# mobilecoinofficial/grapevine

Hardware: AMD Instinct MI355X
Metric: oblivious CRUD req/s (node) at 2^24 msgs, 64K batch; % HBM peak (higher is better)
Workload: dtype u8

## Files before the change

grapevine_amd/csrc/gvs_engine.hip:

```cpp
#include <hip/hip_runtime.h>
#include <rccl/rccl.h>

#include <cmath>
#include <cstdio>
#include <cstdlib>
#include <cstring>
#include <new>
#include <string>
#include <thread>
#include <algorithm>
#include <vector>

#include "../../include/gvstore.h"
#include "../../include/gvstore_test.h"
#include "gvs_kernels.h"
#include "gvs_route.h"
#include "gvs_mtx.h"
#include "gvs_kv.h"
#include "gvs_omap.h"
#include "gvs_wire.h"
#include "gvs_sr25519.h"
#include "gvs_ed25519.h"
#include "gvs_chacha.h"
#include "gvs_spass.h"
// ... 281 lines not shown
    return GVS_ERR_INVALID_ARG;
  if (c->flags & ~(GVS_FLAG_AUTH_STORAGE | GVS_FLAG_ED25519_AUTH)) return GVS_ERR_INVALID_ARG;
  if ((c->flags & GVS_FLAG_AUTH_STORAGE) && c->mailbox_partition_slots > kSrAuth) return GVS_ERR_INVALID_ARG;
  if (c->rows_per_partition && (!is_pow2(c->rows_per_partition) ||
                                c->rows_per_partition < (uint32_t)kTile ||
                                c->rows_per_partition > (uint32_t)kRowsMax))
    return GVS_ERR_INVALID_ARG;
  if (c->shard_count > kShardsMax) return GVS_ERR_INVALID_ARG;
  if (c->route_capacity > c->max_batch) return GVS_ERR_INVALID_ARG;
  for (int i = 0; i < 2; ++i)
    if (c->reserved[i] != 0) return GVS_ERR_INVALID_ARG;
  if (c->expiry_per_batch &&
      (!is_pow2(c->expiry_per_batch) || c->expiry_per_batch > c->max_batch / 2))
    return GVS_ERR_INVALID_ARG;
  return GVS_OK;
}

static uint32_t auto_capacity(uint32_t B, uint32_t S) {
  if (S <= 1) return B;
  const double mu = std::ceil((double)B / S);
  uint64_t c = (uint64_t)std::ceil(mu + 8.0 * std::sqrt(mu) + 64.0);
  c = (c + 63) / 64 * 64;
  return (uint32_t)(c < B ? c : B);
}

static uint32_t shard_batch(uint64_t m) {
  uint64_t p2 = 1024;
  while (p2 < m) p2 <<= 1;
  const uint64_t r = (m + 8191) / 8192 * 8192;
  const uint64_t be = std::max<uint64_t>(1024, std::min(p2, r));
  return be > (1u << (kSeqBits - 1)) ? 0u : (uint32_t)be;
}

static uint32_t txn_slots(uint32_t B, uint32_t W, uint32_t S) {
  const double mu = (double)B / W;
  uint64_t c = (uint64_t)std::ceil(mu + 8.0 * std::sqrt(mu) + 16.0);
  c = (c + 7) / 8 * 8;
  if (c > S) c = S;
  if (c > B) c = B;
  if (c > kSlotMax) c = kSlotMax;
  return (uint32_t)c;
}

static bool expiry_fits(const gvs_config* c, bool sharded) {
  if (!c->expiry_per_batch) return true;
  uint32_t Be = c->max_batch;
  if (sharded) {
    const uint32_t S = c->shard_count ? c->shard_count : 1;
    const uint32_t C = c->route_capacity ? c->route_capacity : auto_capacity(c->max_batch, S);
    Be = shard_batch((uint64_t)S * C + c->expiry_per_batch);
    if (!Be) return false;
  }
  const uint32_t need = txn_slots(c->expiry_per_batch, c->mailbox_partitions, ~0u);
  return need <= txn_slots(Be, c->mailbox_partitions, kGroupMax);
}


static uint8_t gf_mul(uint8_t a, uint8_t b) {
  uint8_t p = 0;
  for (int i = 0; i < 8; ++i) {
    if (b & 1) p ^= a;
    a = (uint8_t)((a << 1) ^ ((a & 0x80) ? 0x1b : 0));
    b >>= 1;
  }
  return p;
}
// ... 93 lines not shown
  for (uint32_t t = 0; t < 4; ++t) sc.l3p[t] = ld32(kb + 1200 + 4 * t);
  sc.nhk = nullptr;
  sc.epoch = 0;
  sc.on = 1;
}

static SealCtx seal_of(const gvs_handle* h, const Engine& e) {
  SealCtx c = h->sc;
  c.epoch = e.epoch;
  return c;
}

static int engine_init(gvs_handle* h, Engine& e, uint32_t shard, uint32_t B) {
  const gvs_config* cfg = &h->cfg;
  e.shard = shard;
  e.N = cfg->msg_capacity;
  e.Q = cfg->mailbox_partitions;
  e.Sr = cfg->mailbox_partition_slots;
  e.R = (uint64_t)e.Q * e.Sr;
  e.B = B;
  e.logQ = log2u(e.Q);
  uint64_t S = cfg->rows_per_partition ? cfg->rows_per_partition : e.N / 4096;
  if (S < (uint64_t)kTile) S = kTile;
  if (S > (uint64_t)kRowsMax) S = kRowsMax;
  if (S > e.N) S = e.N;
  if (!is_pow2(S)) return GVS_ERR_INVALID_ARG;
  e.S = (uint32_t)S;
  e.W = (uint32_t)(e.N / S);
  e.nblk = B / 1024;
  e.ring_size = e.N + B;
  if (e.W + 1 > (uint32_t)kBinsMax) return GVS_ERR_INVALID_ARG;
  e.c = txn_slots(B, e.W, e.S);
  e.cm = txn_slots(B, e.Q, kGroupMax);
  e.X = cfg->expiry_per_batch;
  if (e.X) {
    e.xep = e.X >= e.W ? e.X / e.W : 1u;
    e.xk = e.X >= e.W ? 1u : e.W / e.X;
    if (e.xep > kXepMax) return GVS_ERR_INVALID_ARG;
  }
  e.kc.pk0 = ld64(cfg->secret_key);
  e.kc.pk1 = ld64(cfg->secret_key + 8);
  e.kc.hk0 = ld64(cfg->secret_key + 16);
  e.kc.hk1 = ld64(cfg->secret_key + 24);
  e.kc.tag = shard_tag(shard);
  e.kc.nshards = h->S;

#define A(ptr, n)                                \
  do {                                           \
    if (int r_ = dalloc_t(h, &e.ptr, (n))) return r_; \
  } while (0)
  const uint64_t E = kExtra;
  A(table, e.N * 64);
  A(mbox, e.R * 64);
  A(side, e.R);
  A(ring, e.ring_size);
  A(scal, 1);
  A(img, (B + E) * 64);
  A(types, B);
  A(ops, B);
  A(kinds, B);
  A(s1keys, B);
  A(m1out, B + E);
  A(pflag, B);
  A(pslot, B);
  A(bsum, 2 * e.nblk);
  A(cslot, B);
// ... 164 lines not shown
  h->rt.resize(n_src);
  for (uint32_t k = 0; k < n_eng; ++k) {
    const uint32_t shard = mode == kRccl ? cfg->shard_index : k;
    if (int rc = engine_init(h, h->eng[k], shard, h->Be)) return fail(rc);
  }
  for (uint32_t k = 0; k < n_src; ++k)
    if (int rc = router_init(h, h->rt[k])) return fail(rc);
  const uint64_t stage = (uint64_t)h->Bsub * (mode == kLocal ? h->S : 1u);
  if (int rc = dalloc_t(h, &h->in_stage, stage * kAbiU4)) return fail(rc);
  if (int rc = dalloc_t(h, &h->out_stage, stage * kAbiU4)) return fail(rc);
  if (mode == kRccl) {
    ncclUniqueId id;
    std::memcpy(&id, comm_id, sizeof id);
    ncclResult_t r = ncclCommInitRank(&h->comm, (int)h->S, id, (int)cfg->shard_index);
    if (r != ncclSuccess) {
      h->err = std::string("ncclCommInitRank: ") + ncclGetErrorString(r);
      h->comm = nullptr;
      return fail(GVS_ERR_DEVICE);
    }
  }
  *out = h;
  return GVS_OK;
}


static uint32_t lower_count(uint32_t n, uint32_t blk, uint32_t half) {
  return (n / blk) * half + std::min(n % blk, half);
}

template <typename K, int E>
static void sort_tiles(hipStream_t s, K* d, uint32_t n) {
  constexpr uint32_t L = 1024u * E;
  hipLaunchKernelGGL((k_bitonic_tile<K, E>), dim3(n / L), dim3(1024), 0, s, d, 0u, 1);
  for (uint32_t k = 2 * L; (k >> 1) < n; k <<= 1) {
    uint32_t j = k >> 1;
    for (; j >= 8 * L; j >>= 4) {
      const uint32_t nq = lower_count(n, 2 * j, j >> 3);
      hipLaunchKernelGGL(k_bitonic_global4<K>, dim3((nq + 255) / 256), dim3(256), 0, s, d, n, k, j, nq);
    }
    for (; j >= 2 * L; j >>= 2) {
      const uint32_t nq = lower_count(n, 2 * j, j >> 1);
      hipLaunchKernelGGL(k_bitonic_global2<K>, dim3((nq + 255) / 256), dim3(256), 0, s, d, n, k, j, nq);
    }
    if (j >= L) {
      const uint32_t np = lower_count(n, 2 * j, j);
      hipLaunchKernelGGL(k_bitonic_global<K>, dim3((np + 255) / 256), dim3(256), 0, s, d, n, k, j, np);
    }
    hipLaunchKernelGGL((k_bitonic_tile<K, E>), dim3(n / L), dim3(1024), 0, s, d, k, 0);
  }
}

template <typename K, int EMAX>
static int sort_keys(gvs_handle* h, K* d, uint32_t n) {
  if (n < 1024 || n % 1024) return GVS_ERR_INTERNAL;
  uint32_t e = EMAX;
  while ((n / 1024) % e) e >>= 1;
  switch (e) {
    case 1: sort_tiles<K, 1>(h->stream, d, n); break;
    case 2: sort_tiles<K, 2>(h->stream, d, n); break;
    case 4: sort_tiles<K, (EMAX < 4 ? EMAX : 4)>(h->stream, d, n); break;
    default: sort_tiles<K, EMAX>(h->stream, d, n); break;
  }
  GVS_HIP(h, hipGetLastError());
  return GVS_OK;
}

static MArgs margs(const gvs_handle* h, const Engine& e) {
  MArgs a{};
  a.sc = seal_of(h, e);
  a.te = h->te;
  a.btag = e.btag;
  a.keys = e.s1keys;
  a.mbox = e.mbox;
  a.side = e.side;
  a.m1out = e.m1out;
  a.rop = e.rop;
  a.rres = e.rres;
  a.scal = e.scal;
  a.Q = e.Q;
  a.Sr = e.Sr;
// ... 81 lines not shown

static int phase_a2(gvs_handle* h, Engine& e, const uint4* d_in, uint32_t stride, uint32_t n) {
  hipStream_t s = h->stream;
  const uint32_t B = e.B, nblk = e.nblk;
  e.stamp_run = e.stamp_next++;
  if (e.stamp_next == kNone) e.stamp_next = 1;
  const uint32_t xbase = B - e.X;
  e.gtx = e.gtxb[e.gsel];
  e.gsel ^= 1u;
  const bool fuse = e.m2_pending;
  hipLaunchKernelGGL(k_copy, dim3(B / (4 * kCopyPerWave)), dim3(256), 0, s, d_in, stride, n, B, e.img, e.types,
                     (const uint4*)(e.X ? e.xb2[e.par ^ 1] : nullptr), xbase);
  mark(h, "copy");
  {
    MetaArgs a{e.img, e.types, e.ops, e.kinds, e.s1keys, n, B, e.Q, e.logQ, e.N, e.kc, xbase, e.idn};
    hipLaunchKernelGGL(k_meta, dim3(B / 256), dim3(256), 0, s, a);
  }
  mark(h, "meta");
  if (int r = sort_keys<Key128, 1>(h, e.s1keys, B)) return r;
  mark(h, "sort_s1");
  {
    GtxArgs a{e.s1keys, e.ops, e.mpos, e.gtx, e.gtx_agg, e.gtx_carry, fuse ? e.gscal : e.scal,
              B,        e.Q,   e.logQ, e.cm,  B / kScanT, e.stamp_run};
    a.mpid = e.mpid;
    hipLaunchKernelGGL(k_scan_a<GtxOp>, dim3(B / kScanT), dim3(kScanT), 0, s, a);
    hipLaunchKernelGGL(k_scan_b<GtxOp>, dim3(1), dim3(kScanT), 0, s, a);
    hipLaunchKernelGGL(k_scan_c<GtxOp>, dim3(B / kScanT), dim3(kScanT), 0, s, a);
  }
  mark(h, "gtx");
  if (h->auth) {
    hipLaunchKernelGGL(k_m1a, dim3(e.Q), dim3(256), (e.cm + 1) * sizeof(GroupM) + GVS_MA_EXTRA_LDS, s, margs2(h, e));
  } else if (fuse) {
    M21Args fa{e.m2_args, margs2(h, e), &e.gscal->error};
    hipLaunchKernelGGL(k_m21x, dim3(e.Q), dim3(256), e.Sr * sizeof(uint4) + 2 * (e.cm + 1) * sizeof(GroupM), s,
                       fa);
    hipLaunchKernelGGL(k_err_fold, dim3(1), dim3(64), 0, s, e.scal, &e.gscal->error);
    e.m2_pending = false;
  } else {
    hipLaunchKernelGGL(k_m1x<false>, dim3(e.Q), dim3(256), (e.cm + 1) * sizeof(GroupM), s, margs2(h, e));
  }
  {
    M1rArgs a{};
    vscan_fields(a, e);
    a.mpos = e.mpos;
    a.ops = e.ops;
    a.msnapp = e.msnapp;
    a.mpid = e.mpid;
    a.m1out = e.m1out;
    a.N = e.N;
    a.kc = e.kc;
    vscan_abc<M1rOp>(s, a);
    hipLaunchKernelGGL(k_m1r_c, dim3(a.nvb), dim3(256), 0, s, a);
  }
  mark(h, "m1");
  {
    AllocArgs a = aargs(e);
    hipLaunchKernelGGL(k_alloc_sum, dim3(nblk), dim3(1024), 0, s, a);
    hipLaunchKernelGGL(k_alloc_ring, dim3(1), dim3(1024), 0, s, a);
    hipLaunchKernelGGL(k_alloc_b, dim3(nblk * 4), dim3(256), 0, s, a);
  }
  mark(h, "alloc");
  if (int r = sort_keys<uint64_t, 1>(h, e.rkeys, B)) return r;
  mark(h, "sort_r");
  {
    RtxArgs a{e.rkeys, e.rpos, e.tbuf[e.par], e.rtx_agg, e.rtx_carry, e.scal,
              B,       e.W,    e.S,           e.c,       B / kScanT,  e.stamp_run};
    hipLaunchKernelGGL(k_scan_a<RtxOp>, dim3(B / kScanT), dim3(kScanT), 0, s, a);
    hipLaunchKernelGGL(k_scan_b<RtxOp>, dim3(1), dim3(kScanT), 0, s, a);
// ... 1846 lines not shown

int gvs_store_raw(gvs_handle* h, uint32_t shard, uint32_t region, uint64_t offset,
                  const void* src, uint64_t bytes) {
  if (!h || !src) return GVS_ERR_INVALID_ARG;
  if (int r = flush_m2(h)) return r;
  void* base;
  uint64_t size;
  if (int r = raw_region(h, shard, region, &base, &size)) return r;
  if (offset > size || bytes > size - offset) return GVS_ERR_INVALID_ARG;
  if (const uint32_t tr = tiled(h, region); tr && bytes) {
    const uint64_t tb = (uint64_t)tr * 1024, t0 = offset / tb, t1 = (offset + bytes + tb - 1) / tb;
    std::vector<uint8_t> rows;
    if (int r = tiles_in(h, base, tr, t0, t1 - t0, rows)) return r;
    std::memcpy(&rows[offset - t0 * tb], src, bytes);
    std::vector<uint8_t> t(rows.size());
    for (uint64_t r = 0; r < (t1 - t0) * tr; ++r)
      for (uint32_t b = 0; b < 64; ++b) std::memcpy(&t[tile_u(tr, r, b) * 16], &rows[r * 1024 + b * 16], 16);
    GVS_HIP(h, hipMemcpyAsync((uint8_t*)base + t0 * tb, t.data(), t.size(), hipMemcpyHostToDevice, h->stream));
    GVS_HIP(h, hipStreamSynchronize(h->stream));
    return GVS_OK;
  }
  GVS_HIP(h, hipMemcpyAsync((uint8_t*)base + offset, src, bytes, hipMemcpyHostToDevice, h->stream));
  GVS_HIP(h, hipStreamSynchronize(h->stream));
  return GVS_OK;
}


int gvs_test_set_epoch(gvs_handle* h, uint32_t epoch) {
  if (!h || !h->auth) return GVS_ERR_INVALID_ARG;
  for (auto& e : h->eng) e.epoch = epoch;
  return GVS_OK;
}

gvs_handle* gvs_oram_test_handle(gvs_oram* o) { return o ? o->h : nullptr; }
gvs_handle* gvs_omap_test_handle(gvs_omap* m) { return m ? m->h : nullptr; }

int gvs_route_plan(const gvs_config* cfg, const gvs_request* reqs, uint32_t n, uint32_t* slot,
                   uint32_t* capacity, uint32_t* shard_batch_out, uint8_t* shed) {
  if (!cfg || (n && (!reqs || !slot))) return GVS_ERR_INVALID_ARG;
  if (int rc = validate(cfg)) return rc;
  const uint32_t S = cfg->shard_count ? cfg->shard_count : 1u, B = cfg->max_batch;
  if (n > B) return GVS_ERR_INVALID_ARG;
  const uint32_t C = cfg->route_capacity ? cfg->route_capacity : auto_capacity(B, S);
  RouteArgs a{};
  a.in = reinterpret_cast<const uint4*>(reqs);
  a.n = n;
  a.B = B;
  a.S = S;
  a.C = C;
  a.N = cfg->msg_capacity;
  a.kc.pk0 = ld64(cfg->secret_key);
  a.kc.pk1 = ld64(cfg->secret_key + 8);
  a.kc.hk0 = ld64(cfg->secret_key + 16);
  a.kc.hk1 = ld64(cfg->secret_key + 24);
  a.kc.nshards = S;
  std::vector<uint32_t> cnt(S, 0);
  std::vector<uint64_t> keys(n);
  std::vector<uint32_t> dest(n);
  for (uint32_t i = 0; i < n; ++i) {
    uint32_t k;
    dest[i] = route_dest_key(a, i, k);
    keys[i] = ((uint64_t)k << 32) | i;
  }
  std::sort(keys.begin(), keys.end());
  if (shed) std::fill(shed, shed + n, (uint8_t)0);
  for (uint32_t j = kRouteKeyCap; j < n; ++j) {
// ... 188 lines not shown
```

grapevine_amd/csrc/gvs_kernels.h:

```cpp
#pragma once
#include "gvs_device.h"
#include "gvs_seal_dev.h"

namespace gvs {


template <typename K>
__device__ inline bool key_lt(const K& a, const K& b);
template <>
__device__ inline bool key_lt<uint64_t>(const uint64_t& a, const uint64_t& b) {
  return a < b;
}
template <>
__device__ inline bool key_lt<Key128>(const Key128& a, const Key128& b) {
  return (a.hi < b.hi) | ((a.hi == b.hi) & (a.lo < b.lo));
}

__device__ inline uint64_t key_sel(bool c, uint64_t a, uint64_t b) { return c ? a : b; }
__device__ inline Key128 key_sel(bool c, const Key128& a, const Key128& b) {
  return Key128{c ? a.hi : b.hi, c ? a.lo : b.lo};
}

__device__ inline uint64_t shfl_xor_key(uint64_t a, uint32_t m) {
  const uint32_t lo = __shfl_xor((uint32_t)a, (int)m), hi = __shfl_xor((uint32_t)(a >> 32), (int)m);
// ... 124 lines not shown
  K v[16];
#pragma unroll
  for (uint32_t a = 0; a < 16; ++a) v[a] = data[l[a] ? x[a] : x[0]];
  K t[8];
#pragma unroll
  for (uint32_t a = 0; a < 8; ++a) {
    t[a] = key_sel(flip, v[15 - a], v[8 + a]);
    cx_static(v[a], t[a], flip ? l[15 - a] : l[8 + a]);
  }
#pragma unroll
  for (uint32_t a = 0; a < 8; ++a) v[8 + a] = key_sel(flip, t[7 - a], t[a]);
#pragma unroll
  for (uint32_t s = 4; s >= 1; s >>= 1)
#pragma unroll
    for (uint32_t a = 0; a < 16; ++a)
      if ((a & s) == 0u) cx_static(v[a], v[a + s], l[a + s]);
#pragma unroll
  for (uint32_t a = 0; a < 16; ++a)
    if (l[a]) data[x[a]] = v[a];
}

template <typename K>
__global__ __launch_bounds__(256) void k_bitonic_global(K* data, uint32_t n, uint32_t k,
                                                        uint32_t j, uint32_t np) {
  const uint32_t p = blockIdx.x * blockDim.x + threadIdx.x;
  if (p >= np) return;
  const uint32_t i = ((p / j) * 2u * j) + (p % j);
  const uint32_t pj = (j << 1) == k ? i ^ (2u * j - 1u) : i + j;
  if (pj >= n) return;
  const K a = data[i], b = data[pj];
  const bool sw = key_lt(b, a);
  data[i] = key_sel(sw, b, a);
  data[pj] = key_sel(sw, a, b);
}


__device__ inline uint32_t block1024_prefix(bool f, uint32_t* s_w, uint32_t* total) {
  const uint32_t tid = threadIdx.x, lane = lane_id(), wave = tid >> 6;
  const uint64_t m = __ballot(f);
  if (lane == 0) s_w[wave] = (uint32_t)__popcll(m);
  __syncthreads();
  uint32_t off = 0, tot = 0;
  for (uint32_t w = 0; w < 16; ++w) {
    off += w < wave ? s_w[w] : 0u;
    tot += s_w[w];
  }
  __syncthreads();
  *total = tot;
  return off + mbcnt64(m);
}


constexpr uint32_t kTypeExpire = 0x45585031u;
constexpr uint32_t kCopyPerWave = 8;
__global__ __launch_bounds__(256) void k_copy(const uint4* __restrict__ in, uint32_t stride,
                                              uint32_t n, uint32_t B, uint4* __restrict__ img,
                                              uint32_t* __restrict__ types, const uint4* xbuf,
                                              uint32_t xbase) {
  constexpr uint32_t R = kCopyPerWave;
  const uint32_t i0 = (blockIdx.x * 4 + (threadIdx.x >> 6)) * R;
  const uint32_t lane = lane_id();
  __shared__ uint4 s_rec[4][R * 65];
  if (i0 >= B) return;
  uint4 v[R];
  uint32_t t;
  const uint32_t live = min(n, xbase);
// ... 500 lines not shown
```

grapevine_amd/csrc/gvs_mtx.h:

```cpp
#pragma once
#include "gvs_txn.h"

namespace gvs {


constexpr uint32_t kMPosHead = 1u << 20, kMPosLast = 1u << 21, kMPosNull = 1u << 22;
__host__ __device__ inline uint32_t mpos_cls(uint32_t x) { return (x >> 23) & 3u; }
__host__ __device__ inline uint32_t mpos_sub(uint32_t x) { return (x >> 25) & 1u; }

struct GtxV {
  uint32_t preset, gcnt;
  uint32_t greset, n_next, n_del, n_create, n_x;
  uint32_t fcs, g0, c1;
};

struct GtxArgs {
  const Key128* keys;
  const OpState* ops;
  uint4* mpos;
  uint4* gtx;
  GtxV* agg;
  GtxV* carry;
  Scal* scal;
  uint32_t B, Q, logQ, cm, nblk, stamp;
// ... 700 lines not shown
    const uint32_t nr = nt + spread_lo(ci + 1, nch, dn) - dlo;
    uint32_t mq = mm;
    for (uint32_t r = 0; r < nr; ++r) {
      const uint32_t low = mq & (0u - mq);
      mq &= mq - 1u;
      step(v, mine, low, j0, d0 + dlo + (r - nt));
    }
    if (lane < (uint32_t)kMU && j0 + lane < a.Sr) side[j0 + lane] = mine;
#pragma unroll
    for (int u = 0; u < kMU; ++u) {
      if (j0 + u < a.Sr) st_stream(part, (uint64_t)(j0 + u) * 64 + lane, v[u]);
      va[u] = vb[u];
    }
  }
  if (nch == 0) {
    uint4 v[kMU], mine = make_uint4(0, 0, 0, 0);
#pragma unroll
    for (int u = 0; u < kMU; ++u) v[u] = make_uint4(0, 0, 0, 0);
    for (uint32_t r = 0; r < dn; ++r) step(v, mine, 0u, 0u, d0 + r);
  }
  if (tid == 0)
    atomicAdd((unsigned long long*)&a.scal->n_mailboxes, (unsigned long long)(int64_t)(int32_t)s_delta);
}

#ifndef GVS_DIAG_M21
#define GVS_DIAG_M21 0
#endif

struct M21Args {
  MArgs w, r;
  const uint32_t* gerr;
};

__global__ __launch_bounds__(256) void k_m21x(M21Args A) {
  const MArgs& a = A.w;
  const MArgs& b = A.r;
  extern __shared__ uint4 s_dyn[];
  uint4* s_side = s_dyn;
  GroupM* g = reinterpret_cast<GroupM*>(s_dyn + a.Sr);
  GroupM* g1 = g + a.cm + 1;
  __shared__ int16_t s_sg[kSrMax];
  __shared__ uint8_t s_occb[kSrMax];
  __shared__ uint4 s_wst[4][64];
  __shared__ int16_t s_place[kSrMax];
  __shared__ uint8_t s_flag[kSrMax];
  __shared__ uint16_t s_pfx[kSrMax + 1];
  __shared__ uint16_t s_gpfx[kGroupMax + 1];
  __shared__ uint8_t s_gflag[kGroupMax + 1];
  __shared__ int16_t s_pend[kGroupMax + 1];
  __shared__ uint8_t s_ld[kGroupMax + 1];
  __shared__ uint32_t s_w[4], s_ng, s_occ, s_delta, s_tw[kRowWaves];
  __shared__ int16_t s_sg1[kSrMax];
  __shared__ uint8_t s_occb1[kSrMax];
  __shared__ uint32_t s_ng1, s_occ1, s_empt1, s_tw1[kRowWaves];
  __shared__ uint8_t s_tf1[kGroupMax];
  __shared__ uint16_t s_tp1[kGroupMax + 1];
  __shared__ int16_t s_tl1[kGroupMax];
  const uint32_t tid = threadIdx.x, lane = lane_id();
  const uint32_t wave = __builtin_amdgcn_readfirstlane(tid >> 6);
  const uint32_t q = blockIdx.x;
  if (a.scal->error) return;
  const bool rd = *A.gerr == 0u;
  uint4* part = a.mbox + (uint64_t)q * a.Sr * 64;
  uint4* side = a.side + (uint64_t)q * a.Sr;
  uint4 va[kMU], vb[kMU];
  load_rows(va, part, wave * kMU, a.Sr);
  const uint32_t ng = load_groups(a, q, g, &s_ng, true);
  if (tid == 0) {
    s_occ = 0;
    s_delta = 0;
  }
  __syncthreads();
  side_prepass_m(a, q, g, ng, s_sg, s_occb, &s_occ, s_side);
  __syncthreads();
  for (uint32_t k = tid; k < a.cm; k += 256) {
    GroupM& G = g[k];
    const bool real = k < ng;
    const GroupFields f = group_fields(G);
    const uint32_t len = selu32(real & ((int32_t)f.slot >= 0), f.len, 0u);
    const uint32_t dp = min(G.n_del, len);
    const uint64_t lenmask = len >= 64 ? ~0ull : ((1ull << len) - 1ull);
    const uint64_t mask = (((uint64_t)G.mhi << 32) | G.mlo) & lenmask & ~((1ull << dp) - 1ull);
    const uint32_t nk = len - dp - (uint32_t)__popcll(mask);
    G.fl = selu32(real, nk + min(G.n_succ, GVS_MAILBOX_SLOTS - nk), 0u);
    s_gflag[k] = (real & ((int32_t)f.slot < 0) & (G.fl > 0)) ? 1 : 0;
    s_ld[k] = 0;
  }
  __syncthreads();
  for (uint32_t j = tid; j < a.Sr; j += 256) {
    const int k = s_sg[j];
    const bool occ = s_occb[j] != 0;
    s_flag[j] = (!occ || (k >= 0 && g[k].fl == 0)) ? 1 : 0;
  }
  __syncthreads();
  block_flag_scan(s_flag, a.Sr, s_pfx, s_w);
  block_flag_scan(s_gflag, a.cm, s_gpfx, s_w);
  for (uint32_t k = tid; k < a.cm; k += 256)
    s_pend[s_gflag[k] ? s_gpfx[k] : (uint32_t)kGroupMax] = (int16_t)k;
  __syncthreads();
  const uint32_t npend = s_gpfx[a.cm];
  if (tid == 0 && npend > s_pfx[a.Sr]) atomicOr(&a.scal->error, 2u);
  for (uint32_t j = tid; j < a.Sr; j += 256) {
    const int16_t cand = s_pend[min((uint32_t)s_pfx[j], (uint32_t)kGroupMax)];
    s_place[j] = (s_flag[j] && s_pfx[j] < npend) ? cand : (int16_t)-1;
    const int k = s_sg[j];
    atomicSub(&s_delta, (k >= 0 && g[k >= 0 ? k : 0].fl == 0) ? 1u : 0u);
  }
  if (tid == 0) atomicAdd(&s_delta, npend);
  if (tid < kRowWaves) s_tw[tid] = 0;
  __syncthreads();
  for (uint32_t j = tid; j < a.Sr; j += 256) {
    const int k = s_sg[j], pl = s_place[j];
    const int ge = pl >= 0 ? pl : k;
    s_ld[ge >= 0 ? (uint32_t)ge : (uint32_t)kGroupMax] = 1;
    atomicAdd(&s_tw[(j / kMU) % kRowWaves], ge >= 0 ? 1u : 0u);
  }
  __syncthreads();
  for (uint32_t k = tid; k < a.cm; k += 256) s_gflag[k] = s_ld[k] ? 0 : 1;
  __syncthreads();
  block_flag_scan(s_gflag, a.cm, s_gpfx, s_w);
  for (uint32_t k = tid; k < a.cm; k += 256)
    if (s_gflag[k]) s_pend[s_gpfx[k]] = (int16_t)k;
  __syncthreads();
  const uint32_t nfree = s_gpfx[a.cm];
  for (uint32_t j = tid; j < a.Sr; j += 256) {
    const int k = s_sg[j], pl = s_place[j];
    const int ge = pl >= 0 ? pl : k;
    const GroupM& G = g[ge >= 0 ? (uint32_t)ge : 0u];
    const uint32_t fl = G.fl;
    const uint64_t w1 = (G.glo << 23) | ((uint64_t)fl << 1) | 1ull;
    const uint4 nsd = sel4(fl > 0, make_uint4((uint32_t)G.hi, (uint32_t)(G.hi >> 32), (uint32_t)w1,
                                              (uint32_t)(w1 >> 32)),
                           make_uint4(0, 0, 0, 0));
    s_side[j] = sel4(ge >= 0, nsd, s_side[j]);
  }
  __syncthreads();
  const uint32_t ng1 = load_groups(b, q, g1, &s_ng1, false);
  if (tid == 0) {
    s_occ1 = 0;
    s_empt1 = 0;
  }
  __syncthreads();
  side_prepass_m(b, q, g1, ng1, s_sg1, s_occb1, &s_occ1, nullptr, s_side);
  __syncthreads();
  count_empty(g1, ng1, b.cm, &s_empt1);
  __syncthreads();
  admit_groups(g1, ng1, b.cm, (b.Sr - s_occ1) + s_empt1);
  __syncthreads();
  if (tid < kRowWaves) s_tw1[tid] = 0;
  __syncthreads();
  for (uint32_t j = tid; j < b.Sr; j += 256) atomicAdd(&s_tw1[(j / kMU) % kRowWaves], s_sg1[j] >= 0 ? 1u : 0u);
  for (uint32_t k = tid; k < b.cm; k += 256)
    s_tf1[k] = ((k < ng1) & ((int32_t)group_fields(g1[k]).slot >= 0)) ? 0 : 1;
  __syncthreads();
  block_flag_scan(s_tf1, b.cm, s_tp1, s_w);
  for (uint32_t k = tid; k < b.cm; k += 256)
    if (s_tf1[k]) s_tl1[s_tp1[k]] = (int16_t)k;
  __syncthreads();
  const uint32_t nfree1 = s_tp1[b.cm];
#if GVS_DIAG_M21 == 2
  return;
#endif
  uint32_t d0, dn, e0, en;
  slot_share(s_tw, a.cm, wave, &d0, &dn);
  slot_share(s_tw1, b.cm, wave, &e0, &en);
  const uint32_t nch = a.Sr > wave * kMU ? (a.Sr - wave * kMU + 4 * kMU - 1) / (4 * kMU) : 0u;
  const uint4* res = a.m2tx + (uint64_t)q * a.cm * kVLineU4;
  uint4* dry = a.mdry + (uint64_t)q * kMDryU4;
  uint4* wst = s_wst[wave];
  auto app_src = [&](uint32_t bit, uint32_t j0, uint32_t di) -> const uint4* {
    const bool slot_it = bit == 0u;
    const uint32_t j = j0 + ((uint32_t)__builtin_ctz(bit | (1u << 31)) & 31u);
    const bool listed = slot_it && di < nfree;
    const int k = slot_it ? -1 : s_sg[j], pl = slot_it ? -1 : s_place[j];
    const int ge = slot_it ? (listed ? (int)s_pend[di] : 0) : (pl >= 0 ? pl : k);
    return (slot_it && !listed) ? dry + 256 + 64u * min(di - nfree, 3u)
                                : res + (uint64_t)(ge >= 0 ? ge : 0) * kVLineU4 + 8;
  };
  auto step2 = [&](uint4 (&v)[kMU], uint4& mine, uint32_t bit, uint32_t j0, uint32_t di, uint4 app) {
    const bool slot_it = bit == 0u;
    uint4 cur = v[0];
#pragma unroll
    for (int uu = 1; uu < kMU; ++uu) cur = sel4((bit >> uu) & 1u, v[uu], cur);
    const uint32_t j = j0 + ((uint32_t)__builtin_ctz(bit | (1u << 31)) & 31u);
    const bool listed = slot_it && di < nfree;
    const int k = slot_it ? -1 : s_sg[j], pl = slot_it ? -1 : s_place[j];
    const int ge = slot_it ? (listed ? (int)s_pend[di] : 0) : (pl >= 0 ? pl : k);
    const GroupM& G = g[ge >= 0 ? (uint32_t)ge : 0u];
    const bool matched = pl < 0;
    const uint32_t len = matched ? G.len : 0u;
// ... 92 lines not shown
```

grapevine_amd/store.py:

```python
import ctypes
import os

import numpy as np

from . import abi

_LIB = None
_HERE = os.path.dirname(os.path.abspath(__file__))
_LIB_PATH = os.path.join(_HERE, "libgvstore.so")
_TEST_LIB_PATH = os.path.join(_HERE, "libgvstore_test.so")

EXPORTED = (
    "gvs_config_init", "gvs_create", "gvs_destroy", "gvs_process_batch", "gvs_process_batches",
    "gvs_process_batch_device", "gvs_process_batches_device", "gvs_access", "gvs_get_stats",
    "gvs_synchronize", "gvs_set_option", "gvs_get_option", "gvs_set_timing", "gvs_last_timings", "gvs_last_error", "gvs_version",
    "gvs_comm_unique_id", "gvs_create_sharded", "gvs_storage_seal_row", "gvs_set_expiry_cutoff",
    "gvs_oram_create", "gvs_oram_destroy", "gvs_oram_access_batch", "gvs_oram_access_batch_device",
    "gvs_oram_set_timing", "gvs_oram_last_timings", "gvs_oram_last_error",
    "gvs_omap_create", "gvs_omap_destroy", "gvs_omap_access_batch", "gvs_omap_access_batch_device",
    "gvs_omap_set_timing", "gvs_omap_last_timings", "gvs_omap_last_error",
    "gvs_process_wire_batch", "gvs_process_wire_batch_device", "gvs_wire_decode_device",
    "gvs_wire_encode_device", "gvs_sr25519_verify", "gvs_sr25519_verify_device",
    "gvs_host_alloc", "gvs_host_free", "gvs_process_wire_batches",
    "gvs_ed25519_verify", "gvs_ed25519_verify_device",
    "gvs_challenge_derive", "gvs_challenge_derive_device", "gvs_process_wire_batch_seeded",
    "gvs_process_wire_batch_seeded_device", "gvs_process_wire_batches_seeded",
)
TEST_EXPORTED = ("gvs_dump_messages", "gvs_raw_size", "gvs_dump_raw", "gvs_store_raw",
                 "gvs_route_plan", "gvs_oram_test_handle", "gvs_omap_test_handle", "gvs_test_set_epoch")


def test_hooks_enabled():
    return os.environ.get("GVS_TEST_HOOKS") == "1"


class GvsError(RuntimeError):
    def __init__(self, code, msg):
        super().__init__(f"gvstore error {code}: {msg}")
        self.code = code


def load_library(path=None):
    global _LIB
    if _LIB is not None and path is None:
        return _LIB
    p = path or os.environ.get("GVS_LIB_OVERRIDE") or (_TEST_LIB_PATH if test_hooks_enabled() else _LIB_PATH)
    if not os.path.exists(p):
        raise RuntimeError(f"{os.path.basename(p)} not built at {p}; run `make` (HIP extension missing)")
    lib = ctypes.CDLL(p)
    hooks = hasattr(lib, "gvs_dump_raw")
    vp, u32, i32 = ctypes.c_void_p, ctypes.c_uint32, ctypes.c_int
    lib.gvs_config_init.argtypes = [ctypes.POINTER(abi.GvsConfig), ctypes.c_uint64]
    lib.gvs_create.argtypes = [ctypes.POINTER(abi.GvsConfig), ctypes.POINTER(vp)]
    lib.gvs_comm_unique_id.argtypes = [ctypes.c_char_p]
    lib.gvs_create_sharded.argtypes = [ctypes.POINTER(abi.GvsConfig), ctypes.c_char_p,
                                       ctypes.POINTER(vp)]
    lib.gvs_destroy.argtypes = [vp]
    lib.gvs_process_batch.argtypes = [vp, vp, u32, vp]
    lib.gvs_process_batch_device.argtypes = [vp, vp, u32, vp]
    lib.gvs_process_batches_device.argtypes = [vp, vp, vp, u32, vp, ctypes.POINTER(u32)]
    lib.gvs_process_wire_batch.argtypes = [vp, vp, u32, vp, u32, vp, vp, vp, u32, vp, vp, vp]
    lib.gvs_process_wire_batches.argtypes = [vp, vp, u32, vp, vp, u32, vp, vp, vp, u32, vp, vp,
# ... 7 lines not shown
    lib.gvs_challenge_derive.argtypes = [vp, vp, vp, u32, vp]
    lib.gvs_challenge_derive_device.argtypes = [vp, vp, vp, u32, vp]
    lib.gvs_sr25519_verify.argtypes = [vp, vp, vp, u32, vp, u32, vp, u32, vp]
    lib.gvs_host_alloc.argtypes = [vp, ctypes.c_size_t, ctypes.POINTER(vp)]
    lib.gvs_host_free.argtypes = [vp, vp]
    lib.gvs_sr25519_verify_device.argtypes = [vp, vp, u32, vp, u32, u32, vp, u32, u32, vp, u32, vp]
    lib.gvs_ed25519_verify.argtypes = [vp, vp, vp, u32, vp, u32, vp]
    lib.gvs_ed25519_verify_device.argtypes = [vp, vp, u32, vp, u32, u32, vp, u32, u32, vp]
    lib.gvs_wire_decode_device.argtypes =[vp, vp, u32, vp, u32, vp, vp, vp, vp]
    lib.gvs_wire_encode_device.argtypes = [vp, vp, u32, vp, u32, vp]
    lib.gvs_process_batches.argtypes = [vp, vp, vp, u32, vp, ctypes.POINTER(u32)]
    lib.gvs_access.argtypes = [vp, vp, vp]
    lib.gvs_get_stats.argtypes = [vp, ctypes.POINTER(abi.GvsStats)]
    lib.gvs_synchronize.argtypes = [vp]
    lib.gvs_set_timing.argtypes = [vp, i32]
    lib.gvs_set_option.argtypes = [vp, ctypes.c_char_p, ctypes.c_int64]
    lib.gvs_get_option.argtypes = [vp, ctypes.c_char_p, ctypes.POINTER(ctypes.c_int64)]
    lib.gvs_last_timings.argtypes = [vp, ctypes.POINTER(ctypes.c_char_p),
                                     ctypes.POINTER(ctypes.c_float), i32]
    cp, u64 = ctypes.c_char_p, ctypes.c_uint64
    lib.gvs_storage_seal_row.argtypes = [cp, u32, u64, u32, cp, cp, cp, cp, cp]
    if hooks:
        lib.gvs_dump_messages.argtypes = [vp, vp, ctypes.c_uint64]
        lib.gvs_raw_size.argtypes = [vp, u32, u32, ctypes.POINTER(u64)]
        lib.gvs_dump_raw.argtypes = [vp, u32, u32, u64, vp, u64]
        lib.gvs_store_raw.argtypes = [vp, u32, u32, u64, vp, u64]
        P32 = ctypes.POINTER(u32)
        lib.gvs_route_plan.argtypes = [ctypes.POINTER(abi.GvsConfig), vp, u32, vp, P32, P32, vp]
        lib.gvs_oram_test_handle.argtypes = [vp]
        lib.gvs_oram_test_handle.restype = vp
        lib.gvs_omap_test_handle.argtypes = [vp]
        lib.gvs_omap_test_handle.restype = vp
        lib.gvs_test_set_epoch.argtypes = [vp, u32]
    lib.gvs_last_error.argtypes = [vp]
    lib.gvs_set_expiry_cutoff.argtypes = [vp, ctypes.c_uint64]
    lib.gvs_last_error.restype = ctypes.c_char_p
    lib.gvs_version.restype = ctypes.c_char_p
    lib.gvs_oram_create.argtypes = [ctypes.POINTER(abi.GvsOramConfig), ctypes.POINTER(vp)]
    lib.gvs_oram_destroy.argtypes = [vp]
    lib.gvs_oram_access_batch.argtypes = [vp, vp, u32, vp]
    lib.gvs_oram_access_batch_device.argtypes = [vp, vp, u32, vp]
    lib.gvs_oram_set_timing.argtypes = [vp, i32]
    lib.gvs_oram_last_timings.argtypes = [vp, ctypes.POINTER(ctypes.c_char_p),
                                          ctypes.POINTER(ctypes.c_float), i32]
    lib.gvs_oram_last_error.argtypes = [vp]
    lib.gvs_oram_last_error.restype = ctypes.c_char_p
    lib.gvs_omap_create.argtypes = [ctypes.POINTER(abi.GvsOramConfig), ctypes.POINTER(vp)]
    lib.gvs_omap_destroy.argtypes = [vp]
    lib.gvs_omap_access_batch.argtypes = [vp, vp, u32, vp]
    lib.gvs_omap_access_batch_device.argtypes = [vp, vp, u32, vp]
    lib.gvs_omap_set_timing.argtypes = [vp, i32]
    lib.gvs_omap_last_timings.argtypes = [vp, ctypes.POINTER(ctypes.c_char_p),
                                          ctypes.POINTER(ctypes.c_float), i32]
    lib.gvs_omap_last_error.argtypes = [vp]
    lib.gvs_omap_last_error.restype = ctypes.c_char_p
    for name in EXPORTED + (TEST_EXPORTED if hooks else ()):
        if name not in ("gvs_last_error", "gvs_version", "gvs_oram_last_error", "gvs_omap_last_error",
                        "gvs_oram_test_handle", "gvs_omap_test_handle"):
            getattr(lib, name).restype = i32
    if path is None:
        _LIB = lib
    return lib


def route_plan(config, reqs, with_shed=False):
    lib = load_library(_TEST_LIB_PATH)
# ... 416 lines not shown
```

Measured before the change: 9.430 million.

## Add LDS multi-stride bitonic pass and restructure fused m21 kernel with merged loads and scans

The sort gains a new LDS-based kernel that handles several bitonic strides between the tile size and 64x the tile size in one launch. This replaces multiple global-memory compare-exchange passes. The fused m21x kernel now loads both group tables in one pass and splits the flag scans into begin/finish halves so they overlap other work. It also drops several __syncthreads barriers and uses a wider parallel admit routine. Dynamic LDS above 64KB is opted into via a function attribute, at the risk of lower occupancy and subtle ordering bugs in the barrier-reduced kernel.

New measurement: 9.372 million. About the same (-0.6%).

```diff
diff --git a/grapevine_amd/csrc/gvs_engine.hip b/grapevine_amd/csrc/gvs_engine.hip
--- a/grapevine_amd/csrc/gvs_engine.hip
+++ b/grapevine_amd/csrc/gvs_engine.hip
@@ -337,6 +337,8 @@
   return be > (1u << (kSeqBits - 1)) ? 0u : (uint32_t)be;
 }
 
+static size_t m21_lds(uint32_t Sr, uint32_t cm) { return Sr * sizeof(uint4) + 2 * (size_t)(cm + 1) * sizeof(GroupM); }
+
 static uint32_t txn_slots(uint32_t B, uint32_t W, uint32_t S) {
   const double mu = (double)B / W;
   uint64_t c = (uint64_t)std::ceil(mu + 8.0 * std::sqrt(mu) + 16.0);
@@ -496,6 +498,11 @@
   if (e.W + 1 > (uint32_t)kBinsMax) return GVS_ERR_INVALID_ARG;
   e.c = txn_slots(B, e.W, e.S);
   e.cm = txn_slots(B, e.Q, kGroupMax);
+  if (const size_t lds = m21_lds(e.Sr, e.cm); lds > 65536u && !h->auth && h->kind == 0 &&
+      hipFuncSetAttribute((const void*)k_m21x, hipFuncAttributeMaxDynamicSharedMemorySize, (int)lds) != hipSuccess) {
+    (void)hipGetLastError();
+    return GVS_ERR_INVALID_ARG;
+  }
   e.X = cfg->expiry_per_batch;
   if (e.X) {
     e.xep = e.X >= e.W ? e.X / e.W : 1u;
@@ -726,20 +733,29 @@
 static void sort_tiles(hipStream_t s, K* d, uint32_t n) {
   constexpr uint32_t L = 1024u * E;
   hipLaunchKernelGGL((k_bitonic_tile<K, E>), dim3(n / L), dim3(1024), 0, s, d, 0u, 1);
+  constexpr uint32_t logL = 10u + (E == 1 ? 0u : E == 2 ? 1u : E == 4 ? 2u : 3u);
+  static_assert((1u << logL) == L, "tile size");
+  constexpr uint32_t kCols = 64;
   for (uint32_t k = 2 * L; (k >> 1) < n; k <<= 1) {
     uint32_t j = k >> 1;
-    for (; j >= 8 * L; j >>= 4) {
+    for (; j >= 8 * kCols * L; j >>= 4) {
       const uint32_t nq = lower_count(n, 2 * j, j >> 3);
       hipLaunchKernelGGL(k_bitonic_global4<K>, dim3((nq + 255) / 256), dim3(256), 0, s, d, n, k, j, nq);
     }
-    for (; j >= 2 * L; j >>= 2) {
+    for (; j >= 2 * kCols * L; j >>= 2) {
       const uint32_t nq = lower_count(n, 2 * j, j >> 1);
       hipLaunchKernelGGL(k_bitonic_global2<K>, dim3((nq + 255) / 256), dim3(256), 0, s, d, n, k, j, nq);
     }
-    if (j >= L) {
+    if (j >= kCols * L) {
       const uint32_t np = lower_count(n, 2 * j, j);
       hipLaunchKernelGGL(k_bitonic_global<K>, dim3((np + 255) / 256), dim3(256), 0, s, d, n, k, j, np);
+      j >>= 1;
     }
+    uint32_t logM = 1;
+    while ((L << logM) < 2 * j) ++logM;
+    const uint32_t blocks = (n + 2 * j - 1) / (2 * j), sets = 1u << (logL + logM - 10u);
+    hipLaunchKernelGGL(k_bitonic_global_lds<K>, dim3(blocks * sets), dim3(1024), 0, s, d, n, logM, logL,
+                       (j << 1) == k ? 1u : 0u);
     hipLaunchKernelGGL((k_bitonic_tile<K, E>), dim3(n / L), dim3(1024), 0, s, d, k, 0);
   }
 }
@@ -887,8 +903,7 @@
     hipLaunchKernelGGL(k_m1a, dim3(e.Q), dim3(256), (e.cm + 1) * sizeof(GroupM) + GVS_MA_EXTRA_LDS, s, margs2(h, e));
   } else if (fuse) {
     M21Args fa{e.m2_args, margs2(h, e), &e.gscal->error};
-    hipLaunchKernelGGL(k_m21x, dim3(e.Q), dim3(256), e.Sr * sizeof(uint4) + 2 * (e.cm + 1) * sizeof(GroupM), s,
-                       fa);
+    hipLaunchKernelGGL(k_m21x, dim3(e.Q), dim3(256), m21_lds(e.Sr, e.cm), s, fa);
     hipLaunchKernelGGL(k_err_fold, dim3(1), dim3(64), 0, s, e.scal, &e.gscal->error);
     e.m2_pending = false;
   } else {
@@ -2801,6 +2816,16 @@
   return GVS_OK;
 }
 
+int gvs_test_sort_keys(gvs_handle* h, void* dev_keys, uint32_t n, uint32_t key_bytes) {
+  if (!h || !dev_keys || (key_bytes != 8 && key_bytes != 16)) return GVS_ERR_INVALID_ARG;
+  if (n < 1024 || n % 1024) return GVS_ERR_INVALID_ARG;
+  const int r = key_bytes == 8 ? sort_keys<uint64_t, 1>(h, static_cast<uint64_t*>(dev_keys), n)
+                               : sort_keys<Key128, 1>(h, static_cast<Key128*>(dev_keys), n);
+  if (r) return r;
+  GVS_HIP(h, hipStreamSynchronize(h->stream));
+  return GVS_OK;
+}
+
 gvs_handle* gvs_oram_test_handle(gvs_oram* o) { return o ? o->h : nullptr; }
 gvs_handle* gvs_omap_test_handle(gvs_omap* m) { return m ? m->h : nullptr; }
 
diff --git a/grapevine_amd/csrc/gvs_kernels.h b/grapevine_amd/csrc/gvs_kernels.h
--- a/grapevine_amd/csrc/gvs_kernels.h
+++ b/grapevine_amd/csrc/gvs_kernels.h
@@ -180,6 +180,37 @@
   const bool sw = key_lt(b, a);
   data[i] = key_sel(sw, b, a);
   data[pj] = key_sel(sw, a, b);
+}
+
+template <typename K>
+__global__ __launch_bounds__(1024) void k_bitonic_global_lds(K* data, uint32_t n, uint32_t logM,
+                                                             uint32_t logL, uint32_t mirror) {
+  __shared__ K s[1024];
+  const uint32_t t = threadIdx.x;
+  const uint32_t logC = 10u - logM, C = 1u << logC, M = 1u << logM;
+  const uint32_t sets = 1u << (logL - logC);
+  const uint32_t f = blockIdx.x & (sets - 1u);
+  const uint32_t base = (blockIdx.x >> (logL - logC)) << (logM + logL);
+  const uint32_t c = t >> logC, x = t & (C - 1u);
+  const bool up = (mirror != 0u) & (c >= (M >> 1));
+  const uint32_t ff = up ? sets - 1u - f : f;
+  const uint32_t gi = base + (c << logL) + (ff << logC) + x;
+  const bool live = gi < n;
+  if (live) s[t] = data[gi];
+  __syncthreads();
+  for (uint32_t j = 512u; j >= C; j >>= 1) {
+    if (t < 512u) {
+      const uint32_t i = ((t / j) * 2u * j) + (t % j);
+      const uint32_t pj = ((mirror != 0u) & (j == 512u)) ? i ^ 1023u : i + j;
+      const bool lv = base + ((pj >> logC) << logL) < n;
+      const K a = s[i], b = s[pj];
+      const bool sw = lv & key_lt(b, a);
+      s[i] = key_sel(sw, b, a);
+      s[pj] = key_sel(sw, a, b);
+    }
+    __syncthreads();
+  }
+  if (live) data[gi] = s[t];
 }
 
 
diff --git a/grapevine_amd/csrc/gvs_mtx.h b/grapevine_amd/csrc/gvs_mtx.h
--- a/grapevine_amd/csrc/gvs_mtx.h
+++ b/grapevine_amd/csrc/gvs_mtx.h
@@ -756,6 +756,126 @@
   const uint32_t* gerr;
 };
 
+__device__ inline GroupM group_of_lines(uint4 x, uint4 h, int l0) {
+  const uint4 r0 = x, r1 = shfl4(x, l0 + 1), r2 = shfl4(x, l0 + 2);
+  GroupM G;
+  G.hi = u4lo(r2);
+  G.glo = u4hi(r2);
+  G.n_del = r0.z;
+  G.n_create = r0.w;
+  G.fcs = r1.y;
+  G.len = 0;
+  G.slot = -1;
+  G.flags = 0;
+  G.fl = 0;
+  G.n_succ = h.y;
+  G.mlo = h.z;
+  G.mhi = h.w;
+  G.head = r1.z;
+  G.pad = 0;
+  return G;
+}
+__device__ inline void load_groups_pair(const MArgs& a, const MArgs& b, uint32_t q, GroupM* g, GroupM* g1,
+                                        uint32_t* s_cnt) {
+  const uint32_t lane = lane_id(), wave = threadIdx.x >> 6, sub = lane & 7u;
+  const int l0 = (int)(lane & ~7u);
+  const uint4 zero = make_uint4(0, 0, 0, 0);
+  uint32_t na = 0, nb = 0;
+  for (uint32_t k0 = wave * 8; k0 < a.cm; k0 += 64) {
+    const bool two = k0 + 32 < a.cm;
+    const uint32_t ka = k0 + (lane >> 3), kb = ka + 32;
+    const uint64_t ga = (uint64_t)q * a.cm + min(ka, a.cm - 1u), gb = (uint64_t)q * a.cm + min(kb, a.cm - 1u);
+    const uint4 xa = a.gtx[ga * 8 + sub], ha = a.m2tx[ga * kVLineU4 + sub], ya = b.gtx[ga * 8 + sub];
+    uint4 xb = zero, hb = zero, yb = zero;
+    if (two) {
+      xb = a.gtx[gb * 8 + sub];
+      hb = a.m2tx[gb * kVLineU4 + sub];
+      yb = b.gtx[gb * 8 + sub];
+    }
+    const GroupM Ga = group_of_lines(xa, ha, l0), Ga1 = group_of_lines(ya, zero, l0);
+    const GroupM Gb = group_of_lines(xb, hb, l0), Gb1 = group_of_lines(yb, zero, l0);
+    const bool wa = (sub == 0u) & (ka < a.cm), wb = (sub == 0u) & two & (kb < a.cm);
+    if (wa) {
+      g[ka] = Ga;
+      g1[ka] = Ga1;
+    }
+    if (wb) {
+      g[kb] = Gb;
+      g1[kb] = Gb1;
+    }
+    na += (uint32_t)__popcll(__ballot(wa & (xa.x == a.stamp))) + (uint32_t)__popcll(__ballot(wb & (xb.x == a.stamp)));
+    nb += (uint32_t)__popcll(__ballot(wa & (ya.x == b.stamp))) + (uint32_t)__popcll(__ballot(wb & (yb.x == b.stamp)));
+  }
+  if (lane == 0) {
+    s_cnt[wave] = na;
+    s_cnt[4 + wave] = nb;
+  }
+}
+
+__device__ inline void admit_groups_wide(GroupM* g, uint32_t ng, uint32_t cm, uint32_t freeq) {
+  uint32_t lp = 0;
+  while (lp < 6 && (cm << (lp + 1)) <= 256u) ++lp;
+  const uint32_t P = 1u << lp, per = (cm + P - 1) >> lp;
+  for (uint32_t w0 = 0; w0 < (cm << lp); w0 += 256) {
+    const uint32_t w = w0 + threadIdx.x;
+    const bool own = w < (cm << lp);
+    const uint32_t k = min(w >> lp, cm - 1u), part = w & (P - 1u);
+    GroupM& G = g[k];
+    const GroupFields f = group_fields(G);
+    const bool real = k < ng;
+    const uint32_t len1 = len_after_pops(f, real);
+    const bool exists1 = len1 > 0;
+    const bool isnew = real & !exists1 & (f.n_create > 0);
+    uint32_t rank = 0;
+    for (uint32_t i = 0; i < per; ++i) {
+      const uint32_t k2 = (i << lp) + part;
+      const GroupFields h = group_fields(g[min(k2, cm - 1u)]);
+      const bool r2 = k2 < ng;
+      const uint32_t hl = len_after_pops(h, r2);
+      rank += (r2 & (hl == 0) & (h.n_create > 0) & (h.fcs < f.fcs)) ? 1u : 0u;
+    }
+    for (uint32_t m = 1; m < P; m <<= 1) rank += (uint32_t)__shfl_xor((int)rank, (int)m);
+    if (own & (part == 0u)) {
+      G.fl = len1;
+      G.flags = (exists1 ? 1u : 0u) | ((isnew & (rank < freeq)) ? 2u : 0u);
+    }
+  }
+}
+
+struct FlagScan {
+  uint64_t m[kSrMax / 256];
+};
+__device__ inline FlagScan flag_scan_begin(const uint8_t* flag, uint32_t n, uint32_t* s_wn) {
+  const uint32_t tid = threadIdx.x, lane = lane_id(), wave = tid >> 6;
+  FlagScan fs;
+#pragma unroll
+  for (uint32_t p = 0; p < (uint32_t)kSrMax / 256; ++p) {
+    const uint32_t i = p * 256 + tid;
+    const bool f = i < n && flag[i];
+    fs.m[p] = __ballot(f);
+    if (lane == 0) s_wn[p * 4 + wave] = (uint32_t)__popcll(fs.m[p]);
+  }
+  return fs;
+}
+__device__ inline void flag_scan_finish(const FlagScan& fs, uint32_t n, uint16_t* out, const uint32_t* s_wn) {
+  const uint32_t tid = threadIdx.x, wave = tid >> 6;
+  uint32_t carry = 0;
+#pragma unroll
+  for (uint32_t p = 0; p < (uint32_t)kSrMax / 256; ++p) {
+    uint32_t off = 0, tot = 0;
+#pragma unroll
+    for (uint32_t w = 0; w < 4; ++w) {
+      const uint32_t c = s_wn[p * 4 + w];
+      off += w < wave ? c : 0u;
+      tot += c;
+    }
+    const uint32_t i = p * 256 + tid;
+    if (i < n) out[i] = (uint16_t)(carry + off + mbcnt64(fs.m[p]));
+    carry += tot;
+  }
+  if (tid == 0) out[n] = (uint16_t)carry;
+}
+
 __global__ __launch_bounds__(256) void k_m21x(M21Args A) {
   const MArgs& a = A.w;
   const MArgs& b = A.r;
@@ -773,10 +893,10 @@
   __shared__ uint8_t s_gflag[kGroupMax + 1];
   __shared__ int16_t s_pend[kGroupMax + 1];
   __shared__ uint8_t s_ld[kGroupMax + 1];
-  __shared__ uint32_t s_w[4], s_ng, s_occ, s_delta, s_tw[kRowWaves];
+  __shared__ uint32_t s_wa[16], s_wb[16], s_cnt[8], s_occ, s_delta, s_tw[kRowWaves];
   __shared__ int16_t s_sg1[kSrMax];
   __shared__ uint8_t s_occb1[kSrMax];
-  __shared__ uint32_t s_ng1, s_occ1, s_empt1, s_tw1[kRowWaves];
+  __shared__ uint32_t s_occ1, s_empt1, s_tw1[kRowWaves];
   __shared__ uint8_t s_tf1[kGroupMax];
   __shared__ uint16_t s_tp1[kGroupMax + 1];
   __shared__ int16_t s_tl1[kGroupMax];
@@ -789,13 +909,25 @@
   uint4* side = a.side + (uint64_t)q * a.Sr;
   uint4 va[kMU], vb[kMU];
   load_rows(va, part, wave * kMU, a.Sr);
-  const uint32_t ng = load_groups(a, q, g, &s_ng, true);
+  uint4 sd0 = make_uint4(0, 0, 0, 0);
+  if (wave * 64 < a.Sr) sd0 = side[min(tid, a.Sr - 1u)];
+  load_groups_pair(a, b, q, g, g1, s_cnt);
+  if (tid < a.Sr) s_side[tid] = sd0;
+  for (uint32_t j = 256 + tid; j < a.Sr; j += 256) s_side[j] = side[j];
   if (tid == 0) {
     s_occ = 0;
     s_delta = 0;
-  }
-  __syncthreads();
-  side_prepass_m(a, q, g, ng, s_sg, s_occb, &s_occ, s_side);
+    s_occ1 = 0;
+    s_empt1 = 0;
+  }
+  if (tid < kRowWaves) {
+    s_tw[tid] = 0;
+    s_tw1[tid] = 0;
+  }
+  __syncthreads();
+  const uint32_t ng = s_cnt[0] + s_cnt[1] + s_cnt[2] + s_cnt[3];
+  const uint32_t ng1 = s_cnt[4] + s_cnt[5] + s_cnt[6] + s_cnt[7];
+  side_prepass_m(a, q, g, ng, s_sg, s_occb, &s_occ, nullptr, s_side);
   __syncthreads();
   for (uint32_t k = tid; k < a.cm; k += 256) {
     GroupM& G = g[k];
@@ -817,8 +949,12 @@
     s_flag[j] = (!occ || (k >= 0 && g[k].fl == 0)) ? 1 : 0;
   }
   __syncthreads();
-  block_flag_scan(s_flag, a.Sr, s_pfx, s_w);
-  block_flag_scan(s_gflag, a.cm, s_gpfx, s_w);
+  {
+    const FlagScan fr = flag_scan_begin(s_flag, a.Sr, s_wa), fg = flag_scan_begin(s_gflag, a.cm, s_wb);
+    __syncthreads();
+    flag_scan_finish(fr, a.Sr, s_pfx, s_wa);
+    flag_scan_finish(fg, a.cm, s_gpfx, s_wb);
+  }
   for (uint32_t k = tid; k < a.cm; k += 256)
     s_pend[s_gflag[k] ? s_gpfx[k] : (uint32_t)kGroupMax] = (int16_t)k;
   __syncthreads();
@@ -826,30 +962,13 @@
   if (tid == 0 && npend > s_pfx[a.Sr]) atomicOr(&a.scal->error, 2u);
   for (uint32_t j = tid; j < a.Sr; j += 256) {
     const int16_t cand = s_pend[min((uint32_t)s_pfx[j], (uint32_t)kGroupMax)];
-    s_place[j] = (s_flag[j] && s_pfx[j] < npend) ? cand : (int16_t)-1;
+    const int pl = (s_flag[j] && s_pfx[j] < npend) ? cand : (int16_t)-1;
+    s_place[j] = (int16_t)pl;
     const int k = s_sg[j];
     atomicSub(&s_delta, (k >= 0 && g[k >= 0 ? k : 0].fl == 0) ? 1u : 0u);
-  }
-  if (tid == 0) atomicAdd(&s_delta, npend);
-  if (tid < kRowWaves) s_tw[tid] = 0;
-  __syncthreads();
-  for (uint32_t j = tid; j < a.Sr; j += 256) {
-    const int k = s_sg[j], pl = s_place[j];
     const int ge = pl >= 0 ? pl : k;
     s_ld[ge >= 0 ? (uint32_t)ge : (uint32_t)kGroupMax] = 1;
     atomicAdd(&s_tw[(j / kMU) % kRowWaves], ge >= 0 ? 1u : 0u);
-  }
-  __syncthreads();
-  for (uint32_t k = tid; k < a.cm; k += 256) s_gflag[k] = s_ld[k] ? 0 : 1;
-  __syncthreads();
-  block_flag_scan(s_gflag, a.cm, s_gpfx, s_w);
-  for (uint32_t k = tid; k < a.cm; k += 256)
-    if (s_gflag[k]) s_pend[s_gpfx[k]] = (int16_t)k;
-  __syncthreads();
-  const uint32_t nfree = s_gpfx[a.cm];
-  for (uint32_t j = tid; j < a.Sr; j += 256) {
-    const int k = s_sg[j], pl = s_place[j];
-    const int ge = pl >= 0 ? pl : k;
     const GroupM& G = g[ge >= 0 ? (uint32_t)ge : 0u];
     const uint32_t fl = G.fl;
     const uint64_t w1 = (G.glo << 23) | ((uint64_t)fl << 1) | 1ull;
@@ -858,28 +977,26 @@
                            make_uint4(0, 0, 0, 0));
     s_side[j] = sel4(ge >= 0, nsd, s_side[j]);
   }
-  __syncthreads();
-  const uint32_t ng1 = load_groups(b, q, g1, &s_ng1, false);
-  if (tid == 0) {
-    s_occ1 = 0;
-    s_empt1 = 0;
-  }
-  __syncthreads();
+  if (tid == 0) atomicAdd(&s_delta, npend);
+  __syncthreads();
+  for (uint32_t k = tid; k < a.cm; k += 256) s_gflag[k] = s_ld[k] ? 0 : 1;
+  const FlagScan ff = flag_scan_begin(s_gflag, a.cm, s_wb);
   side_prepass_m(b, q, g1, ng1, s_sg1, s_occb1, &s_occ1, nullptr, s_side);
   __syncthreads();
+  flag_scan_finish(ff, a.cm, s_gpfx, s_wb);
+  for (uint32_t k = tid; k < a.cm; k += 256)
+    if (s_gflag[k]) s_pend[s_gpfx[k]] = (int16_t)k;
   count_empty(g1, ng1, b.cm, &s_empt1);
-  __syncthreads();
-  admit_groups(g1, ng1, b.cm, (b.Sr - s_occ1) + s_empt1);
-  __syncthreads();
-  if (tid < kRowWaves) s_tw1[tid] = 0;
-  __syncthreads();
   for (uint32_t j = tid; j < b.Sr; j += 256) atomicAdd(&s_tw1[(j / kMU) % kRowWaves], s_sg1[j] >= 0 ? 1u : 0u);
   for (uint32_t k = tid; k < b.cm; k += 256)
     s_tf1[k] = ((k < ng1) & ((int32_t)group_fields(g1[k]).slot >= 0)) ? 0 : 1;
-  __syncthreads();
-  block_flag_scan(s_tf1, b.cm, s_tp1, s_w);
+  const FlagScan ft = flag_scan_begin(s_tf1, b.cm, s_wa);
+  __syncthreads();
+  const uint32_t nfree = s_gpfx[a.cm];
+  flag_scan_finish(ft, b.cm, s_tp1, s_wa);
   for (uint32_t k = tid; k < b.cm; k += 256)
     if (s_tf1[k]) s_tl1[s_tp1[k]] = (int16_t)k;
+  admit_groups_wide(g1, ng1, b.cm, (b.Sr - s_occ1) + s_empt1);
   __syncthreads();
   const uint32_t nfree1 = s_tp1[b.cm];
 #if GVS_DIAG_M21 == 2
diff --git a/grapevine_amd/store.py b/grapevine_amd/store.py
--- a/grapevine_amd/store.py
+++ b/grapevine_amd/store.py
@@ -27,7 +27,8 @@
     "gvs_process_wire_batch_seeded_device", "gvs_process_wire_batches_seeded",
 )
 TEST_EXPORTED = ("gvs_dump_messages", "gvs_raw_size", "gvs_dump_raw", "gvs_store_raw",
-                 "gvs_route_plan", "gvs_oram_test_handle", "gvs_omap_test_handle", "gvs_test_set_epoch")
+                 "gvs_route_plan", "gvs_oram_test_handle", "gvs_omap_test_handle", "gvs_test_set_epoch",
+                 "gvs_test_sort_keys")
 
 
 def test_hooks_enabled():
@@ -101,6 +102,7 @@
         lib.gvs_omap_test_handle.argtypes = [vp]
         lib.gvs_omap_test_handle.restype = vp
         lib.gvs_test_set_epoch.argtypes = [vp, u32]
+        lib.gvs_test_sort_keys.argtypes = [vp, vp, u32, u32]
     lib.gvs_last_error.argtypes = [vp]
     lib.gvs_set_expiry_cutoff.argtypes = [vp, ctypes.c_uint64]
     lib.gvs_last_error.restype = ctypes.c_char_p
```
